# CODEJIN/multi_speaker_tts

Measured on AMD Instinct MI355X. Metric: mel-frames/sec (train step) at batch 32x(128 tok,800 mel), higher is better.
Workload: dtype f32

## Files before the change

multi_speaker_tts_amd/csrc/persist.hip:

```cpp
#include "persist_fwd_parts.h"

namespace mstts {

#ifndef M1_LATE
#define M1_LATE 60
#endif
#ifndef PRE_EARLY
#define PRE_EARLY 1
#endif
#ifndef SPLIT_M0
#define SPLIT_M0 1
#endif
#ifndef SPLIT_C0
#define SPLIT_C0 1
#endif

#ifndef FWD_QOWN
#define FWD_QOWN 1
#endif
#ifndef SPLIT_H1
#define SPLIT_H1 1
#endif
#ifndef SPLIT_H0
#define SPLIT_H0 1
#endif
#ifndef QP_LATE
#define QP_LATE 1
#endif
#ifndef QP_SLEEP
#define QP_SLEEP 12
#endif
#ifndef H0_LATE
#define H0_LATE 1
#endif
#ifndef H1_REQ_EARLY
#define H1_REQ_EARLY 1
#endif
#ifndef P0_EARLY
#define P0_EARLY 0
#endif

constexpr long XCTX = 8L * 128 * 24, XACT = 8L * 128 * 32, XPART = 256L * 8 * 2 * 256, XM1 = 32L * PH, XEN = 32L * 8 * PTMAX;
constexpr long OFF_CTX = 0, OFF_M0 = OFF_CTX + PRING * XCTX, OFF_H0 = OFF_M0 + PRING * XACT, OFF_H1 = OFF_H0 + PRING * XACT,
               OFF_M1 = OFF_H1 + PRING * XACT, OFF_EN = OFF_M1 + PRING * XM1, OFF_P0 = OFF_EN + PRING * XEN, OFF_P1 = OFF_P0 + PRING * XPART,
               OFF_QP = OFF_P1 + PRING * XPART, XQP = 32L * 8 * 256 * 16,
               XCH_FLOATS = OFF_QP + (FWD_QOWN ? PRING * XQP : 0);
template <int TT> struct FL {
    static constexpr int S_STG = 0, S_RED = S_STG + (TT == 128 ? 3 * 128 * 32 / 2 : 128 * LA),
                         S_TR = S_RED + 4 * 2 * 256, S_M1 = S_TR + 2 * 128,
                         S_EN = TT > 128 ? S_STG : S_M1 + PH, S_CUM = TT > 128 ? S_M1 + PH : S_EN + 8 * PT,
                         S_A = S_CUM + TT + 48, S_Q = S_A + TT, S_QF = S_Q + 512, S_CO = S_QF + 16, S_LK = S_CO + 4 * 96,
                         S_FLAG = S_LK + 32 * 16, S_STAMP = S_FLAG + 4, S_VAL = S_STAMP + 2 * 16, S_WQ = S_VAL + PT * 96, S_FLOATS = S_WQ + 8 * 512 * 4;
    static_assert(8 * TT <= 128 * LA && S_FLOATS * 4 <= 160 * 1024, "LDS budget");
};
constexpr int NSTAMP = 16;

struct PersistFwd {
    const float* w0pk; const float* w1pk; const float* wqpk;
    const float* xw0; const float* b1;
    const float* pre; const float* b0;
    const uint8_t* zc0; const uint8_t* zh0; const uint8_t* zc1; const uint8_t* zh1; float keep;
    const float* keys; const float* values; const int32_t* lengths;
    const float* loc_k; const float* loc_b; const float* score_w; const float* score_b;
    int B, S, T;
    float* in0; float* in1; float* pj; float* c0; float* c1; float* acts0; float* acts1; float* craw0; float* craw1;
    float* q_hist; float* align_hist; float* cum_hist;
    float* opk;
    float* xch; unsigned* ctrl;
    unsigned long long* stamps;
    int fail_step; int near_xcd;
};


template <bool PROF, bool FOLD, int TT, bool BF16 = false>
__global__ __launch_bounds__(PTH) void persist_fwd_kernel(PersistFwd d) {
    static_assert(!BF16 || FOLD, "the bf16 instantiation forms the prenet rows' product itself");
    constexpr bool SM0 = SPLIT_M0 && !BF16 && FOLD && TT == 128;
    constexpr bool PE = PRE_EARLY && SPLIT_M0 && SPLIT_C0 && !BF16 && FOLD && TT == 128;
    constexpr bool SC0 = SPLIT_C0 && SM0;
    constexpr bool QO = FWD_QOWN && SC0, SH1 = SPLIT_H1 && QO, SH0 = SPLIT_H0 && QO;
    constexpr int S_BIA = FL<TT>::S_Q + 128;
    typedef FL<TT> Y;
    constexpr int S_STG = Y::S_STG, S_RED = Y::S_RED, S_TR = Y::S_TR, S_M1 = Y::S_M1, S_EN = Y::S_EN, S_CUM = Y::S_CUM, S_A = Y::S_A, S_Q = Y::S_Q,
                  S_CO = Y::S_CO, S_LK = Y::S_LK, S_FLAG = Y::S_FLAG, S_STAMP = Y::S_STAMP, S_VAL = Y::S_VAL, S_WQ = Y::S_WQ;
    constexpr int S_WQO = S_M1, S_W1LO = S_WQ, S_W0LO = S_WQ + 4 * 512 * 4;
    constexpr int NH = TT / 128;
    extern __shared__ __attribute__((aligned(16))) float sm[];
    const int g0 = blockIdx.x, tid0 = threadIdx.x, wave0 = __builtin_amdgcn_readfirstlane(tid0 >> 6);
    int g = g0, gi = g & 7, gj = g >> 3;
    int tid = tid0, lane = tid & 63, wave = wave0;
    const int B = d.B, S = d.S, T = d.T;
    const __amdgpu_buffer_rsrc_t xr = __builtin_amdgcn_make_buffer_rsrc(d.xch, 0, (int)(XCH_FLOATS * 4), 0x00020000);
    unsigned* sflag = reinterpret_cast<unsigned*>(sm + S_FLAG);
    float* stg = sm + S_STG;
    __bf16* stg16 = reinterpret_cast<__bf16*>(sm + S_STG);

    if (d.near_xcd) persist_scrub(xr, OFF_CTX, OFF_M1 - OFF_CTX, g0, tid);
    __syncthreads();
    if (tid == 0) {
// ... 23 lines not shown
    }
    pbf16x8 w1s[SM0 ? 3 : 1][SM0 ? 4 : 1];
    pbf16x8 w0s[SC0 ? 3 : 1][SC0 ? 4 : 1];
    if constexpr (SM0) {
        const float* p1 = d.w1pk + ((long)(g * 8 + wave) * 64) * 64 + lane;
        const float* p0 = d.w0pk + ((long)(g * 8 + wave) * 64) * 64 + lane;
#pragma unroll
        for (int r = 0; r < 32; ++r) {
            {
                const float x = p1[r * 64];
                const __bf16 hi = (__bf16)x; const float r1 = x - (float)hi;
                const __bf16 mid = (__bf16)r1; const float r2 = r1 - (float)mid;
                w1s[0][r >> 3][r & 7] = hi; w1s[1][r >> 3][r & 7] = mid; w1s[2][r >> 3][r & 7] = (__bf16)r2;
            }
            if constexpr (SC0) {
                const float x = p0[r * 64];
                const __bf16 hi = (__bf16)x; const float r1 = x - (float)hi;
                const __bf16 mid = (__bf16)r1; const float r2 = r1 - (float)mid;
                w0s[0][r >> 3][r & 7] = hi; w0s[1][r >> 3][r & 7] = mid; w0s[2][r >> 3][r & 7] = (__bf16)r2;
            }
        }
    }
    pbf16x8 w1h[SH1 ? 2 : 1][SH1 ? 4 : 1];
    pbf16x8 w0h[SH0 ? 2 : 1][SH0 ? 4 : 1];
    if constexpr (SH1 || SH0) {
        const float* p1 = d.w1pk + ((long)(g * 8 + wave) * 64) * 64 + lane;
        const float* p0 = d.w0pk + ((long)(g * 8 + wave) * 64) * 64 + lane;
#pragma unroll
        for (int j = 0; j < 4; ++j) {
            pbf16x8 lo1, lo0;
#pragma unroll
// ... 15 lines not shown
            if constexpr (SH0) *reinterpret_cast<pbf16x8*>(sm + S_W0LO + (j * PTH + tid) * 4) = lo0;
        }
    }
    int ab = gj;
    const bool arow = ab < B;
    const int alen = arow ? (d.lengths ? d.lengths[ab] : T) : 0;
    int ak = tid & 15, atg = tid >> 4;
    float kreg[4 * NH];
    float asb = 0.f, awk = 0.f;
    {
#pragma unroll
        for (int m = 0; m < 4 * NH; ++m) {
            const int t = 128 * (m >> 2) + 4 * atg + (m & 3);
            kreg[m] = (arow && t < T) ? d.keys[((long)ab * T + t) * PA + 16 * gi + ak] : 0.f;
        }
        asb = d.score_b[16 * gi + ak] + d.loc_b[16 * gi + ak];
        awk = d.score_w[16 * gi + ak];
        if constexpr (SC0) {
            if (tid < 16) { sm[S_BIA + 32 + tid] = asb; sm[S_BIA + 48 + tid] = awk; }
            if (tid < 32) {
                const int q = (tid >> 2) & 3, u = 4 * g + (tid & 3);
                sm[S_BIA + tid] = (tid < 16) ? d.b0[q * PH + u] : d.b1[q * PH + u];
            }
        }
        for (int x = tid; x < 32 * 16; x += PTH) sm[S_LK + x] = (x < PKS * 16) ? d.loc_k[(x >> 4) * PA + 16 * gi + (x & 15)] : 0.f;
        for (int x = tid; x < PT * 96; x += PTH) {
            const int t = x / 96, c = x - t * 96;
            sm[S_VAL + x] = (arow && t < alen && t < T) ? d.values[((long)ab * T + t) * PM + 96 * gi + c] : 0.f;
        }
        for (int x = tid; x < TT + 48; x += PTH) sm[S_CUM + x] = 0.f;
        if constexpr (QO) {
            if (tid < 128) {
                const pf32x4 v = reinterpret_cast<const pf32x4*>(d.wqpk)[((long)(tid >> 4) * 8 + gi) * 512 + 16 * gj + (tid & 15)];
#pragma unroll
                for (int u = 0; u < 4; ++u) sm[S_WQO + u * 128 + tid] = v[u];
            }
        } else {
            const pf32x4* wqs = reinterpret_cast<const pf32x4*>(d.wqpk) + (long)gi * 8 * 512;
            for (int x = tid; x < 8 * 512; x += PTH) {
                pf32x4 v = wqs[x];
                if constexpr (BF16) { v[0] = bf16_round(v[0]); v[1] = bf16_round(v[1]); v[2] = bf16_round(v[2]); v[3] = bf16_round(v[3]); }
                reinterpret_cast<pf32x4*>(sm + S_WQ)[x] = v;
            }
// ... 29 lines not shown
    if (wave < 4) {                                                                                                             \
        _Pragma("unroll") for (int m = 0; m < 4; ++m)                                                                           \
            poff[m] = (unsigned)(((OFFP) + slot * XPART + (((long)g * 8 + 2 * wave + (m >> 1)) * 2 + (m & 1)) * 256) * 4 + 16 * lane); \
        issue<4>(xr, poff, pv);                                                                                                 \
    }
#define COMPLETE_PARTIALS()                                                                                                     \
    if (wave < 4) {                                                                                                             \
        const unsigned gens__[4] = {gen, gen, gen, gen};                                                                        \
        if (!complete<4>(xr, poff, pv, d.ctrl, gens__)) PFAIL();                                                                        \
        *reinterpret_cast<pf32x4*>(sm + S_RED + ((wave * 2 + 0) * 64 + lane) * 4) = pv[0] + pv[2];                              \
        *reinterpret_cast<pf32x4*>(sm + S_RED + ((wave * 2 + 1) * 64 + lane) * 4) = pv[1] + pv[3];                              \
    }
#define SUM_PARTIALS()                                                                                                          \
    ((*reinterpret_cast<const pf32x4*>(sm + S_RED + ((0 * 2 + et) * 64 + lane) * 4) + *reinterpret_cast<const pf32x4*>(sm + S_RED + ((1 * 2 + et) * 64 + lane) * 4)) + \
     (*reinterpret_cast<const pf32x4*>(sm + S_RED + ((2 * 2 + et) * 64 + lane) * 4) + *reinterpret_cast<const pf32x4*>(sm + S_RED + ((3 * 2 + et) * 64 + lane) * 4)))
    __syncthreads();
    if (PROF && tid == 0) sflag[2] = (unsigned)wall_clock64();

    float xwv[4] = {0.f, 0.f, 0.f, 0.f};
    pf32x4 prv = {0.f, 0.f, 0.f, 0.f};
    uint8_t zc0v, zh0v, zc1v, zh1v;
#define PL_TID (QO ? tid : tid0)
#define PL_WAVE (QO ? wave : wave0)
#define PL_G (QO ? g : g0)
#define LOAD_PRE(ST) do { const long bp__ = (long)(ST) * B;                                                                                  \
            const unsigned rho__ = ((unsigned)PL_TID & 255u) >> 1, pb__ = 16 * ((rho__ >> 4) & 1u) + (rho__ & 15u);                                     \
            const pf32x4 v__ = *reinterpret_cast<const pf32x4*>(d.pre + (bp__ + (pb__ < (unsigned)B ? pb__ : 0u)) * 256 + 32 * (PL_G & 7) + 8 * (rho__ >> 5) + 4 * ((unsigned)PL_TID & 1u)); \
            prv = pb__ < (unsigned)B ? v__ : (pf32x4){0.f, 0.f, 0.f, 0.f}; } while (0)
#define LOAD_OPERANDS(ST) do { const long b__ = (long)(ST) * B; const unsigned r__ = (16 * (PL_WAVE & 1) + (PL_TID & 15)) < (unsigned)B ? 16 * (PL_WAVE & 1) + (PL_TID & 15) : 0u;  \
         \
// ... 33 lines not shown
                __syncthreads();
                mfma_part_bf16<3, 4, 0>(wb0, stg16, lane, acc0);
            } else if constexpr (SC0) {
                if (!PE || s == 0) {
                    if (tid < 256) sp3_put_rk(stg16, tid >> 1, 6 + (tid & 1), prv);
                    __syncthreads();
                    mfma_part_split3<3, 4>(w0s, stg16, lane, acc0);
                }
            } else {
                if (tid < 256) *reinterpret_cast<pf32x4*>(stg + (tid >> 1) * LA + 24 + 4 * (tid & 1)) = prv;
                __syncthreads();
                mfma_part<6, 8, LA, 0, 64>(w0, stg, lane, acc0);
            }
            if (s > 0) {
                PSTAMP(0);
                slice_issue<6>(xr, OFF_CTX + pslot * XCTX + gi * 3072L, tid, soff, sv);
                if constexpr (BF16) { if (!slice_complete_bf16<6>(xr, stg16, tid, soff, sv, d.ctrl, pgen)) PFAIL(); }
                else if constexpr (SC0) { if (!slice_complete_split3_k6(xr, stg16, tid, soff, sv, d.ctrl, pgen)) PFAIL(); }
                else { if (!slice_complete<6, LA>(xr, stg, tid, soff, sv, d.ctrl, pgen)) PFAIL(); }
                PABORT_CHECK();
                PSTAMP(1);
                if constexpr (BF16) mfma_part_bf16<0, 3, 0>(wb0, stg16, lane, acc0);
                else if constexpr (SC0) mfma_part_split3<0, 3>(w0s, stg16, lane, acc0);
                else mfma_part<0, 6, LA, 0, 64>(w0, stg, lane, acc0);
            }
        } else {
            if (s > 0) {
                PSTAMP(0);
                slice_issue<6>(xr, OFF_CTX + pslot * XCTX + gi * 3072L, tid, soff, sv);
                if (!slice_complete<6, LC>(xr, stg, tid, soff, sv, d.ctrl, pgen)) PFAIL();
                PABORT_CHECK();
                PSTAMP(1);
            }
            if constexpr (!BF16) { if (s > 0) mfma_part<0, 6, LC, 0, 64>(w0, stg, lane, acc0); }
        }
        if constexpr (SH1 && H1_REQ_EARLY) { if (s > 0) slice_issue<8>(xr, OFF_H1 + pslot * XACT + gi * 4096L, tid, soff, sv); }
        PUBLISH_PARTIAL(OFF_P0, acc0)
        PSTAMP(2);
        if (s > 0) {
            if constexpr (!(SH1 && H1_REQ_EARLY)) slice_issue<8>(xr, OFF_H1 + pslot * XACT + gi * 4096L, tid, soff, sv);
            __syncthreads();
            if constexpr (BF16) { if (!slice_complete_bf16<8>(xr, stg16, tid, soff, sv, d.ctrl, pgen)) PFAIL(); }
            else if constexpr (SH1) { if (!slice_complete_split3(xr, stg16, tid, soff, sv, d.ctrl, pgen)) PFAIL(); }
            else { if (!slice_complete<8, LA>(xr, stg, tid, soff, sv, d.ctrl, pgen)) PFAIL(); }
            PABORT_CHECK();
            if constexpr (SH1 && P0_EARLY) { ISSUE_PARTIALS(OFF_P0) }
            if constexpr (BF16) mfma_part_bf16<0, 4, 4>(wb1, stg16, lane, acc1);
            else if constexpr (SH1) mfma_part_split3_lds<0, 4>(w1h, sm + S_W1LO + 4 * tid, stg16, lane, acc1);
            else mfma_part<0, 8, LA, 32, 64>(w1, stg, lane, acc1);
        }
        PSTAMP(13);
        if (!(SH1 && P0_EARLY) || s == 0) { ISSUE_PARTIALS(OFF_P0) }
        COMPLETE_PARTIALS()
        PABORT_CHECK();
        PSTAMP(3);
        {
            const pf32x4 gs = SUM_PARTIALS();
            float add0[4];
#pragma unroll
            for (int q = 0; q < 4; ++q) add0[q] = SC0 ? sm[S_BIA + q * 4 + ee] : FOLD ? b0v[q] : (rowok ? xwv[q] : 0.f);
            const float cprev0 = c0s;
            const CellOut o = cell_update(gs, add0, c0s, h0s, (zc0v || !rowok) ? d.keep : 0.f, (zh0v || !rowok) ? d.keep : 0.f);
            if (ew) {
                sm[S_TR + er * 4 + ee] = o.m;
                sm[S_TR + 128 + er * 4 + ee] = h0s;
            }
            __syncthreads();
            if (tid < 64) {
                const int arr = tid >> 5, row = tid & 31;
                const pf32x4 val = *reinterpret_cast<const pf32x4*>(sm + S_TR + arr * 128 + row * 4);
                const int rho = (((gj & 3) * 2 + (row >> 4)) * 16) + (row & 15);
                const long base = arr ? OFF_H0 : OFF_M0;
                const long o2 = gi * 4096L + rho * 32 + 4 * (gj >> 2);
                xpublish_near(xr, (unsigned)((base + slot * XACT + o2) * 4), val, gen, near);
            }
// ... 161 lines not shown
                if (lane < 16) sm[S_Q + wave * 16 + lane] = qp;
            }
            }
            __syncthreads();
            float qsum = 0.f;
#pragma unroll
            for (int u = 0; u < 8; ++u) qsum += sm[S_Q + u * 16 + ak];
            if (tid < 16) (d.q_hist + (sB + ab) * PA + 16 * gi)[tid] = qsum;
            {
                const float qk = qsum + (SC0 ? sm[S_BIA + 32 + ak] : asb);
#pragma unroll
                for (int hh = 0; hh < NH; ++hh) {
                    const pf32x4 loc = locv[hh];
                    float pre[4];
#pragma unroll
                    for (int m = 0; m < 4; ++m) pre[m] = kreg[4 * hh + m] + qk + loc[m];
                    pf32x4 e4;
#pragma unroll
                    for (int m = 0; m < 4; ++m) {
                        float e = (SC0 ? sm[S_BIA + 48 + ak] : awk) * tanhf_(pre[m]);
                        e += dpp_mov<0xB1, 0xf>(0.f, e);
                        e += dpp_mov<0x4E, 0xf>(0.f, e);
                        e += dpp_mov<0x141, 0xf>(0.f, e);
                        e += dpp_mov<0x140, 0xf>(0.f, e);
                        e4[m] = e;
                    }
                    if (ak == 0) {
                        const long o = ((long)ab * 8 + gi) * TT + 128 * hh + 4 * atg;
                        xpublish(xr, (unsigned)((OFF_EN + slot * XEN + o) * 4), e4, gen);
                    }
                }
// ... 31 lines not shown
                mx = wave_max(mx);
                float ps = 0.f;
#pragma unroll
                for (int i = 0; i < 2 * NH; ++i) { ev[i] = (lane + 64 * i < alen) ? __expf(ev[i] - mx) : 0.f; ps += ev[i]; }
                const float inv = 1.f / wave_sum(ps);
                float* ah = d.align_hist + (sB + ab) * T; float* ch = d.cum_hist + (sB1 + ab) * T;
#pragma unroll
                for (int i = 0; i < 2 * NH; ++i) {
                    const float a = ev[i] * inv, n = sm[S_CUM + 15 + 64 * i + lane] + a;
                    sm[S_A + 64 * i + lane] = a;
                    sm[S_CUM + 15 + 64 * i + lane] = n;
                    if (gi == 0 && lane + 64 * i < T) { ah[lane + 64 * i] = a; ch[lane + 64 * i] = n; }
                }
            }
            __syncthreads();
            if (tid < 384) {
                const int c = tid % 96, th = tid / 96;
                float acc = 0.f;
#pragma unroll
                for (int t4 = 0; t4 < 8; ++t4) {
                    const pf32x4 a4 = *reinterpret_cast<const pf32x4*>(sm + S_A + 32 * th + 4 * t4);
#pragma unroll
                    for (int e = 0; e < 4; ++e) acc += a4[e] * sm[S_VAL + (32 * th + 4 * t4 + e) * 96 + c];
                }
                if (NH > 1) {
                    const float* vg = d.values + ((long)ab * T + 128 + 32 * th) * PM + 96 * gi + c;
                    const int nt = T - (128 + 32 * th) < 32 ? (T - (128 + 32 * th) > 0 ? T - (128 + 32 * th) : 0) : 32;
#pragma unroll 16
                    for (int t = 0; t < 32; ++t) acc += sm[S_A + 128 + 32 * th + t] * (t < nt ? vg[(long)t * PM] : 0.f);
                }
                sm[S_CO + th * 96 + c] = acc;
            }
            __syncthreads();
            if (tid < 24) {
                const pf32x4 val = (*reinterpret_cast<const pf32x4*>(sm + S_CO + 4 * tid) + *reinterpret_cast<const pf32x4*>(sm + S_CO + 96 + 4 * tid)) +
                                   (*reinterpret_cast<const pf32x4*>(sm + S_CO + 192 + 4 * tid) + *reinterpret_cast<const pf32x4*>(sm + S_CO + 288 + 4 * tid));
                const int qq = tid / 6, k4 = tid - qq * 6;
                const int rho = ((qq * 2 + (ab >> 4)) * 16) + (ab & 15);
                const long o = gi * 3072L + rho * 24 + 4 * k4;
                xpublish_near(xr, (unsigned)((OFF_CTX + slot * XCTX + o) * 4), val, gen, near);
                reinterpret_cast<pf32x4*>(d.in0 + (sB1 + ab) * (PM + PH) + 96 * gi)[tid] = val;
                reinterpret_cast<pf32x4*>(d.pj + (sB + ab) * (PH + PM) + PH + 96 * gi)[tid] = val;
            }
        } else {
            PSTAMP(14);
            if (tid < 24) {
                const int qq = tid / 6, k4 = tid - qq * 6;
                const int rho = ((qq * 2 + (ab >> 4)) * 16) + (ab & 15);
                const long o = gi * 3072L + rho * 24 + 4 * k4;
                xpublish_near(xr, (unsigned)((OFF_CTX + slot * XCTX + o) * 4), (pf32x4){0.f, 0.f, 0.f, 0.f}, gen, near);
            }
        }
        PSTAMP(15);
        LOAD_OPERANDS(s + 1 < S ? s + 1 : s);
    }
    if (tid == 0) {
        __hip_atomic_fetch_add(d.ctrl + 2, 1u, __ATOMIC_RELAXED, __HIP_MEMORY_SCOPE_AGENT);
        if (PROF && d.stamps) {
#pragma unroll
            for (int x = 0; x < NSTAMP; ++x) d.stamps[(long)g * NSTAMP + x] = sstamp[x];
        }
    }
#undef PSTAMP
#undef LOAD_OPERANDS
#undef LOAD_PRE
#undef PL_TID
#undef PL_WAVE
#undef PL_G
#undef PABORT_CHECK
#undef PFAIL
#undef PUBLISH_PARTIAL
#undef ISSUE_PARTIALS
#undef COMPLETE_PARTIALS
#undef SUM_PARTIALS
}


__global__ void persist_pack_cells_kernel(const float* __restrict__ w0f, const float* __restrict__ w1, const float* __restrict__ wx0, float* __restrict__ w0pk, float* __restrict__ w1pk) {
    const long n0 = 256L * 8 * 64 * 64, n1 = 256L * 8 * 64 * 64;
    for (long p = blockIdx.x * (long)blockDim.x + threadIdx.x; p < n0 + n1; p += (long)gridDim.x * blockDim.x) {
        const bool c1 = p >= n0;
        long r = c1 ? p - n0 : p;
        const int lane = (int)(r & 63); r >>= 6;
        const int ks = (int)(r & 63); r >>= 6;
        const int wave = (int)(r & 7), g = (int)(r >> 3);
        const int gi = g & 7, gj = g >> 3;
        const int q = lane >> 4, mcol = lane & 15, ue = mcol >> 2, gate = mcol & 3;
        const int u = 32 * gj + 4 * wave + ue;
        const long col = (long)gate * PH + u;
        long row;
        if (!c1) row = ks < 24 ? 96 * gi + 24 * q + ks : ks < 32 ? 32 * gi + 8 * q + (ks - 24) : PM + unit_of_kstep(gi, ks - 32, q);
        else row = ks < 32 ? unit_of_kstep(gi, ks, q) : PH + unit_of_kstep(gi, ks - 32, q);
        if (c1) w1pk[p - n0] = w1[row * 4 * PH + col];
        else w0pk[p] = (ks >= 24 && ks < 32) ? (wx0 ? wx0[row * 4 * PH + col] : 0.f) : w0f[row * 4 * PH + col];
    }
}
__global__ void persist_pack_wq_kernel(const float* __restrict__ wq, float* __restrict__ wqpk) {
    const int p = blockIdx.x * blockDim.x + threadIdx.x;
    if (p >= 8 * 64 * 256) return;
    const int e = p & 3, tid = (p >> 2) & 511, x4 = (p >> 11) & 7, gi = p >> 14;
    wqpk[p] = wq[(long)(32 * (tid >> 4) + 4 * x4 + e) * PA + 16 * gi + (tid & 15)];
}

}
using namespace mstts;

#define PFW_INST(P_, F_, T_, B16_) {persist_fwd_kernel<P_, F_, T_, B16_>, (int)(FL<T_>::S_FLOATS * 4)}
#define PFW_FORMS(T_)                                                                                                                  \
    PFW_INST(false, false, T_, false), PFW_INST(true, false, T_, false), PFW_INST(false, true, T_, false), PFW_INST(true, true, T_, false), \
    PFW_INST(false, true, T_, true), PFW_INST(true, true, T_, true)
static const PersistInst<PersistFwd> FWD_TABLE[] = {PFW_FORMS(128), PFW_FORMS(256)};
#undef PFW_FORMS
#undef PFW_INST
constexpr int fwd_index(bool t256, int form, bool stamps) { return (t256 * 3 + form) * 2 + stamps; }
static_assert(sizeof(FWD_TABLE) / sizeof(FWD_TABLE[0]) == fwd_index(true, 2, true) + 1, "one table row per (positions, form, stamps)");

extern "C" int64_t mstts_persist_fwd_ws_bytes(void) { return XCH_FLOATS * 4; }
extern "C" int64_t mstts_persist_pack_floats(int32_t which) { return which == 0 ? 256L * 8 * 64 * 64 : which == 1 ? 256L * 8 * 64 * 64 : 8L * 64 * 256; }

extern "C" int32_t mstts_persist_fwd_supported(int64_t B, int64_t H, int64_t M, int64_t A, int64_t T, int64_t KS) {
    if (!(B >= 1 && B <= PROWS && H == PH && M == PM && A == PA && T >= 1 && T <= PTMAX && KS == PKS)) return 0;
    static int memo[PERSIST_MAX_DEVICES];
    return persist_device_memo(memo, [](int dev) { return persist_probe(dev, FWD_TABLE); });
}

extern "C" int mstts_persist_pack(const float* w0f, const float* w1, const float* wq, const float* wx0, float* w0pk, float* w1pk, float* wqpk, mstts_stream_t s) {
    MSTTS_REQUIRE(w0f && w1 && wq && w0pk && w1pk && wqpk, MSTTS_ERR_SHAPE, "persist_pack: null pointer");
    hipLaunchKernelGGL(persist_pack_cells_kernel, dim3(4096), dim3(256), 0, (hipStream_t)s, w0f, w1, wx0, w0pk, w1pk);
    MSTTS_CHECK_LAUNCH("persist_pack_cells");
    hipLaunchKernelGGL(persist_pack_wq_kernel, dim3(8 * 64), dim3(256), 0, (hipStream_t)s, wq, wqpk);
    MSTTS_CHECK_LAUNCH("persist_pack_wq");
    return MSTTS_OK;
}

extern "C" int mstts_decoder_train_fwd_persistent(const mstts_decoder_train_desc* d, const mstts_persist_desc* p, mstts_stream_t s) {
    const bool fold = p && p->pre != nullptr;
    MSTTS_REQUIRE(d && p && (fold ? p->b0 != nullptr : d->xw0 != nullptr) && d->b1 && d->in0 && d->in1 && d->pj && d->c0 && d->c1 && d->acts0 && d->acts1 && d->craw0 && d->craw1 &&
                  d->q_hist && d->align_hist && d->cum_hist && p->w0pk && p->w1pk && p->wqpk && p->xch && p->ctrl, MSTTS_ERR_SHAPE,
                  "decoder_train_fwd_persistent: null pointer");
    const long B = d->B, S = d->S, H = d->H, M = d->lsa.M, A = d->lsa.A, T = d->lsa.T;
    MSTTS_REQUIRE(d->lsa.B == B && mstts_persist_fwd_supported(B, H, M, A, T, d->lsa.KS), MSTTS_ERR_SHAPE,
                  "decoder_train_fwd_persistent: shape or device not supported (see mstts_persist_fwd_supported)");
    MSTTS_REQUIRE(d->zc0 && d->zh0 && d->zc1 && d->zh1, MSTTS_ERR_SHAPE, "decoder_train_fwd_persistent: the four zoneout keep-masks are required (all ones = no zoneout)");
    MSTTS_REQUIRE(d->lsa.keys && d->lsa.values && d->lsa.loc_k && d->lsa.loc_b && d->lsa.score_w && d->lsa.score_b, MSTTS_ERR_SHAPE,
                  "decoder_train_fwd_persistent: attention constants missing");
    MSTTS_REQUIRE(aligned16(p->xch) && aligned16(d->in0) && aligned16(d->pj) && (M + H) % 4 == 0, MSTTS_ERR_ALIGN, "decoder_train_fwd_persistent: 16-byte alignment");
    hipStream_t hs = (hipStream_t)s;
    hipError_t e = hipMemsetAsync(d->in0, 0, B * (M + H) * sizeof(float), hs);
    if (e == hipSuccess) e = hipMemsetAsync(d->in1, 0, B * 2 * H * sizeof(float), hs);
    if (e == hipSuccess) e = hipMemsetAsync(d->c0, 0, B * H * sizeof(float), hs);
    if (e == hipSuccess) e = hipMemsetAsync(d->c1, 0, B * H * sizeof(float), hs);
    if (e == hipSuccess) e = hipMemsetAsync(d->cum_hist, 0, B * T * sizeof(float), hs);
    if (e != hipSuccess) return set_err(MSTTS_ERR_LAUNCH, "decoder_train_fwd_persistent: memset: %s", hipGetErrorString(e));
    if (int r = persist_arm("decoder_train_fwd_persistent", p->xch, XCH_FLOATS * 4, p->ctrl, PCTRL_WORDS, hs)) return r;
    PersistFwd a;
    MSTTS_REQUIRE(!fold || (d->P == 256 && aligned16(p->pre)), MSTTS_ERR_SHAPE, "decoder_train_fwd_persistent: the folded prenet product needs a 256-wide prenet, 16-byte aligned");
    a.w0pk = p->w0pk; a.w1pk = p->w1pk; a.wqpk = p->wqpk; a.xw0 = d->xw0; a.b1 = d->b1; a.pre = p->pre; a.b0 = p->b0;
    a.zc0 = d->zc0; a.zh0 = d->zh0; a.zc1 = d->zc1; a.zh1 = d->zh1; a.keep = 1.f - d->zoneout;
    a.keys = d->lsa.keys; a.values = d->lsa.values; a.lengths = d->lsa.lengths;
    a.loc_k = d->lsa.loc_k; a.loc_b = d->lsa.loc_b; a.score_w = d->lsa.score_w; a.score_b = d->lsa.score_b;
    a.B = (int)B; a.S = (int)S; a.T = (int)T;
    a.in0 = d->in0; a.in1 = d->in1; a.pj = d->pj; a.c0 = d->c0; a.c1 = d->c1; a.acts0 = d->acts0; a.acts1 = d->acts1;
    a.craw0 = d->craw0; a.craw1 = d->craw1; a.q_hist = d->q_hist; a.align_hist = d->align_hist; a.cum_hist = d->cum_hist;
    a.opk = p->opk; a.xch = p->xch; a.ctrl = p->ctrl; a.stamps = (unsigned long long*)p->stamps;
    persist_knobs(a, p->selftest_fail_step, p->near_xcd);
    MSTTS_REQUIRE(!p->recurrent_bf16 || fold, MSTTS_ERR_SHAPE, "decoder_train_fwd_persistent: the bf16 form needs the folded prenet product (pre / b0)");
    const PersistInst<PersistFwd>& k = FWD_TABLE[fwd_index(T > 128, p->recurrent_bf16 ? 2 : fold ? 1 : 0, p->stamps != nullptr)];
    hipLaunchKernelGGL(k.kernel, dim3(PWG), dim3(PTH), (size_t)k.lds_bytes, hs, a);
    MSTTS_CHECK_LAUNCH("persist_fwd");
    return MSTTS_OK;
}
```

multi_speaker_tts_amd/csrc/persist_fwd_parts.h:

```cpp
#pragma once
#include "persist_common.h"
#include "lstm_cell.h"

namespace mstts {

constexpr int LC = 28, LA = 36;

template <int K4A, int K4B, int LD, int WOFF, int NW, int NT = 2>
__device__ __forceinline__ void mfma_part(const float (&w)[NW], const float* sx, int lane, pf32x4 (&acc)[2]) {
    const int row0 = ((lane >> 4) * 2) * 16 + (lane & 15);
#pragma unroll
    for (int k4 = K4A; k4 < K4B; ++k4) {
        const pf32x4 x0 = *reinterpret_cast<const pf32x4*>(sx + row0 * LD + 4 * k4);
        if (NT == 2) {
            const pf32x4 x1 = *reinterpret_cast<const pf32x4*>(sx + (row0 + 16) * LD + 4 * k4);
#pragma unroll
            for (int e = 0; e < 4; ++e) {
                acc[0] = PMFMA(w[WOFF + 4 * k4 + e], x0[e], acc[0]);
                acc[1] = PMFMA(w[WOFF + 4 * k4 + e], x1[e], acc[1]);
            }
        } else {
#pragma unroll
            for (int e = 0; e < 4; ++e) acc[0] = PMFMA(w[WOFF + 4 * k4 + e], x0[e], acc[0]);
        }
// ... 82 lines not shown
}
__device__ __forceinline__ bool slice_complete_split3(__amdgpu_buffer_rsrc_t xr, __bf16* stg, int tid, const unsigned (&off)[2], pf32x4 (&v)[2], const unsigned* ctrl, unsigned gen) {
    const unsigned gens[2] = {gen, gen};
    const bool ok = complete<2>(xr, off, v, ctrl, gens);
    sp3_put(stg, tid, v[0]);
    sp3_put(stg, tid + PTH, v[1]);
    return ok;
}
__device__ __forceinline__ bool slice_complete_split3_k6(__amdgpu_buffer_rsrc_t xr, __bf16* stg, int tid, const unsigned (&off)[2], pf32x4 (&v)[2], const unsigned* ctrl, unsigned gen) {
    const unsigned gens[2] = {gen, gen};
    const bool ok = complete<2>(xr, off, v, ctrl, gens);
    { const int rho = tid / 6; sp3_put_rk(stg, rho, tid - rho * 6, v[0]); }
    if (tid + PTH < 128 * 6) { const int p = tid + PTH, rho = p / 6; sp3_put_rk(stg, rho, p - rho * 6, v[1]); }
    return ok;
}
template <int JA = 0, int JB = 4>
__device__ __forceinline__ void mfma_part_split3(const pbf16x8 (&wsp)[3][4], const __bf16* sx, int lane, pf32x4 (&acc)[2]) {
    const int row0 = ((lane >> 4) * 2) * 16 + (lane & 15);
#pragma unroll
    for (int j = JA; j < JB; ++j) {
#pragma unroll
        for (int t = 0; t < 2; ++t) {
            const __bf16* p = sx + sp3_off(row0 + 16 * t, j);
            const pbf16x8 xh = *reinterpret_cast<const pbf16x8*>(p), xm = *reinterpret_cast<const pbf16x8*>(p + SP3_PLANE),
                          xl = *reinterpret_cast<const pbf16x8*>(p + 2 * SP3_PLANE);
            acc[t] = PMFMA_BF16(wsp[0][j], xh, acc[t]);
            acc[t] = PMFMA_BF16(wsp[1][j], xh, acc[t]);
            acc[t] = PMFMA_BF16(wsp[0][j], xm, acc[t]);
            acc[t] = PMFMA_BF16(wsp[1][j], xm, acc[t]);
            acc[t] = PMFMA_BF16(wsp[2][j], xh, acc[t]);
// ... 40 lines not shown
```

multi_speaker_tts_amd/engine.py:

```python
from __future__ import annotations

import ctypes as C
import os
import types
import warnings

import numpy as np
import torch

from . import lib
from .lib import ACT_NONE, ACT_RELU, ACT_TANH, gemm, ptr, call
from .masks import MaskSet, step_seed
from .params import CELL, ENC_CELL, LSA, LSA_VARS, VOC, Dims, ParamStore, bank_groups, bank_suffix
from .persist import PERSIST_COOLDOWN, PERSIST_STRIKES, CoolDown, Ticket, decoder_workgroups, lstm_bwd_workgroups, lstm_fwd_workgroups, near_xcd
from .training import (BN_EPS, BN_MOM, Engine, _split_k, _split_k_big, bn_train_fwd, conv_bn_bwd, conv_fwd, exponential_decay, lstm_layer_grads,
                       lstm_seq_bwd, lstm_seq_fwd)

MAX_PLANS = 64


def learning_rate(step):
    from . import Hyper_Parameters as hp
    return exponential_decay(hp.Train.Learning_Rate, step)

# ... 368 lines not shown
        w.d_pj = f(S, B, H + M, zero=bool(self.ctx_dead))
        w.dg0, w.dg1 = f(S, B, 4 * H), f(S, B, 4 * H)
        w.dq_hist, w.de_hist = f(S, B, A), f(S, B, Te)
        w.d_in0_parts = int(lb.mstts_decoder_train_bwd_parts(H, M))
        w.d_in0 = f(w.d_in0_parts, S, B, M + H, zero=bool(self.ctx_dead))
        w.dec_bwd_ws = f(int(lb.mstts_decoder_train_bwd_ws_floats(B, H, M, A, Te, d.att_ch)), zero=True)
        w.lsa_param_ws = f((int(lb.mstts_lsa_param_bwd_ws_floats(B, Te, S)) + 3) // 4 * 4)
        w.d_pre, w.d_pre2 = f(S * B, Pn), f(S * B, Pn)
        w.d_keys, w.d_values = f(B, Te, A), f(B, Te, M, zero=bool(self.ctx_dead))
        w.enc_dgs, w.enc_dgp = {dr: f(Te, B, 4 * He) for dr in ("fw", "bw")}, {dr: f(B, Te, 4 * He) for dr in ("fw", "bw")}
        w.enc_bwd_ws = {dr: f(int(lb.mstts_lstm_seq_ws_floats(B, He, 1))) for dr in ("fw", "bw")}
        w.enc_dy, w.enc_dz, w.enc_dx = f(B * Te, max(d.enc_conv_ch, d.emb)), f(B * Te, d.enc_conv_ch), f(B * Te, max(d.enc_conv_ch, d.emb))
        w.job_flag, w.job_flag_host = cv.take(1, dtype=torch.int32), self._pin("job_flag_host", 1)
        w.dec, w.dec_b = lib.DecoderTrain(), lib.DecoderTrainBwd()
        w.dec_b.ctx_dead = self.ctx_dead
        if w.persist_bwd:
            w.pdesc_b.ctx_dead = self.ctx_dead
        w.zero_on_activate, w.extent_bytes, w.arena_generation = cv.zero, cv.off, self._arena.generation
        return (None if (cv.count or cv.overflow) else w), cv.off

    def _forward_plan(self, w, batch, masks, allowed, overlap_vocoder, redo):
        allowed = False if redo else (self._persist_begin_step() if allowed is None else bool(allowed))
        decoder, bptt, encoder = bool(w.persist) and allowed, bool(w.persist_bwd) and allowed, bool(w.persist_enc) and allowed
        return types.SimpleNamespace(
            decoder=decoder,
            bptt=bptt,
            packed_bptt=decoder and bptt,
            encoder=encoder,
            encoder_forked=encoder and ENC_OVERLAP,
            late_masks=masks is None and encoder and ENC_OVERLAP,
# ... 612 lines not shown
```

Baseline: 669,500.

## Specialize persistent decoder forward for constant dead context columns

When the last 256 value channels are constant over time (ctx_dead), a new kernel instantiation computes the attention context only over the live channels. A small pre-kernel folds the dead channels' contribution into a per-batch cell-0 gate constant, and another kernel fills the dead columns of in0/pj. This shrinks the per-step context exchange and MFMA work, and the change also enables early partial issue with an 8-wave reduction layout. In exchange it adds two launches, extra LDS use for keys and the constant, and a more complex weight-loading path.

```diff
diff --git a/multi_speaker_tts_amd/csrc/persist.hip b/multi_speaker_tts_amd/csrc/persist.hip
--- a/multi_speaker_tts_amd/csrc/persist.hip
+++ b/multi_speaker_tts_amd/csrc/persist.hip
@@ -37,8 +37,9 @@
 #define H1_REQ_EARLY 1
 #endif
 #ifndef P0_EARLY
-#define P0_EARLY 0
-#endif
+#define P0_EARLY 2
+#endif
+constexpr bool FWD_LIVE_BUILT = FWD_QOWN && SPLIT_C0 && SPLIT_M0;
 
 constexpr long XCTX = 8L * 128 * 24, XACT = 8L * 128 * 32, XPART = 256L * 8 * 2 * 256, XM1 = 32L * PH, XEN = 32L * 8 * PTMAX;
 constexpr long OFF_CTX = 0, OFF_M0 = OFF_CTX + PRING * XCTX, OFF_H0 = OFF_M0 + PRING * XACT, OFF_H1 = OFF_H0 + PRING * XACT,
@@ -61,6 +62,7 @@
     const float* pre; const float* b0;
     const uint8_t* zc0; const uint8_t* zh0; const uint8_t* zc1; const uint8_t* zh1; float keep;
     const float* keys; const float* values; const int32_t* lengths;
+    const float* cst;
     const float* loc_k; const float* loc_b; const float* score_w; const float* score_b;
     int B, S, T;
     float* in0; float* in1; float* pj; float* c0; float* c1; float* acts0; float* acts1; float* craw0; float* craw1;
@@ -72,17 +74,23 @@
 };
 
 
-template <bool PROF, bool FOLD, int TT, bool BF16 = false>
+template <bool PROF, bool FOLD, int TT, bool BF16 = false, int MC = PM>
 __global__ __launch_bounds__(PTH) void persist_fwd_kernel(PersistFwd d) {
     static_assert(!BF16 || FOLD, "the bf16 instantiation forms the prenet rows' product itself");
+    constexpr bool LIVE = MC != PM;
+    constexpr int CW = MC / 8, K4C = CW / 16;
+    static_assert(MC == PM || (MC == PM - 256 && FWD_LIVE_BUILT && !BF16 && FOLD && TT == 128), "live width: the fp32 / folded / 128-position instantiation only");
     constexpr bool SM0 = SPLIT_M0 && !BF16 && FOLD && TT == 128;
     constexpr bool PE = PRE_EARLY && SPLIT_M0 && SPLIT_C0 && !BF16 && FOLD && TT == 128;
     constexpr bool SC0 = SPLIT_C0 && SM0;
     constexpr bool QO = FWD_QOWN && SC0, SH1 = SPLIT_H1 && QO, SH0 = SPLIT_H0 && QO;
+    constexpr bool P0E = P0_EARLY && SH1 && LIVE, P0E8 = P0E && P0_EARLY == 2;
     constexpr int S_BIA = FL<TT>::S_Q + 128;
     typedef FL<TT> Y;
     constexpr int S_STG = Y::S_STG, S_RED = Y::S_RED, S_TR = Y::S_TR, S_M1 = Y::S_M1, S_EN = Y::S_EN, S_CUM = Y::S_CUM, S_A = Y::S_A, S_Q = Y::S_Q,
                   S_CO = Y::S_CO, S_LK = Y::S_LK, S_FLAG = Y::S_FLAG, S_STAMP = Y::S_STAMP, S_VAL = Y::S_VAL, S_WQ = Y::S_WQ;
+    constexpr int S_KEY = S_VAL + PT * CW;
+    constexpr int S_CST = S_M1 + 512;
     constexpr int S_WQO = S_M1, S_W1LO = S_WQ, S_W0LO = S_WQ + 4 * 512 * 4;
     constexpr int NH = TT / 128;
     extern __shared__ __attribute__((aligned(16))) float sm[];
@@ -136,7 +144,9 @@
                 w1s[0][r >> 3][r & 7] = hi; w1s[1][r >> 3][r & 7] = mid; w1s[2][r >> 3][r & 7] = (__bf16)r2;
             }
             if constexpr (SC0) {
-                const float x = p0[r * 64];
+                const int crow = 64 * gi + 16 * (lane >> 4) + r, ci = crow / 96, cq = (crow - 96 * ci) / 24, ck = crow - 96 * ci - 24 * cq;
+                const float x = (!LIVE || r >= 24) ? p0[r * 64] : r >= 16 ? 0.f
+                              : d.w0pk[((long)((gj * 8 + ci) * 8 + wave) * 64 + ck) * 64 + 16 * cq + (lane & 15)];
                 const __bf16 hi = (__bf16)x; const float r1 = x - (float)hi;
                 const __bf16 mid = (__bf16)r1; const float r2 = r1 - (float)mid;
                 w0s[0][r >> 3][r & 7] = hi; w0s[1][r >> 3][r & 7] = mid; w0s[2][r >> 3][r & 7] = (__bf16)r2;
@@ -182,6 +192,7 @@
             const int t = 128 * (m >> 2) + 4 * atg + (m & 3);
             kreg[m] = (arow && t < T) ? d.keys[((long)ab * T + t) * PA + 16 * gi + ak] : 0.f;
         }
+        if constexpr (LIVE) *reinterpret_cast<pf32x4*>(sm + S_KEY + 4 * tid) = (pf32x4){kreg[0], kreg[1], kreg[2], kreg[3]};
         asb = d.score_b[16 * gi + ak] + d.loc_b[16 * gi + ak];
         awk = d.score_w[16 * gi + ak];
         if constexpr (SC0) {
@@ -192,9 +203,13 @@
             }
         }
         for (int x = tid; x < 32 * 16; x += PTH) sm[S_LK + x] = (x < PKS * 16) ? d.loc_k[(x >> 4) * PA + 16 * gi + (x & 15)] : 0.f;
-        for (int x = tid; x < PT * 96; x += PTH) {
-            const int t = x / 96, c = x - t * 96;
-            sm[S_VAL + x] = (arow && t < alen && t < T) ? d.values[((long)ab * T + t) * PM + 96 * gi + c] : 0.f;
+        for (int x = tid; x < PT * CW; x += PTH) {
+            const int t = x / CW, c = x - t * CW;
+            sm[S_VAL + x] = (arow && t < alen && t < T) ? d.values[((long)ab * T + t) * PM + CW * gi + c] : 0.f;
+        }
+        if constexpr (LIVE) {
+            const int r = tid & 31;
+            sm[S_CST + tid] = r < B ? d.cst[(long)r * 4 * PH + (tid >> 7) * PH + 4 * g + ((tid >> 5) & 3)] : 0.f;
         }
         for (int x = tid; x < TT + 48; x += PTH) sm[S_CUM + x] = 0.f;
         if constexpr (QO) {
@@ -254,6 +269,19 @@
 #define SUM_PARTIALS()                                                                                                          \
     ((*reinterpret_cast<const pf32x4*>(sm + S_RED + ((0 * 2 + et) * 64 + lane) * 4) + *reinterpret_cast<const pf32x4*>(sm + S_RED + ((1 * 2 + et) * 64 + lane) * 4)) + \
      (*reinterpret_cast<const pf32x4*>(sm + S_RED + ((2 * 2 + et) * 64 + lane) * 4) + *reinterpret_cast<const pf32x4*>(sm + S_RED + ((3 * 2 + et) * 64 + lane) * 4)))
+#define S_RED8(W) ((W) < 4 ? S_RED + (W) * 512 : S_KEY + 2048 + ((W) - 4) * 512)
+#define ISSUE_PARTIALS8(OFFP) do {                                                                                              \
+        _Pragma("unroll") for (int m = 0; m < 2; ++m)                                                                           \
+            soff[m] = (unsigned)(((OFFP) + slot * XPART + (((long)g * 8 + wave) * 2 + m) * 256) * 4 + 16 * lane);               \
+        issue<2>(xr, soff, sv); } while (0)
+#define COMPLETE_PARTIALS8() do {                                                                                               \
+        const unsigned gens__[2] = {gen, gen};                                                                                  \
+        if (!complete<2>(xr, soff, sv, d.ctrl, gens__)) PFAIL();                                                                \
+        float* red__ = sm + (wave < 4 ? S_RED + wave * 512 : S_KEY + 2048 + (wave - 4) * 512);                                  \
+        *reinterpret_cast<pf32x4*>(red__ + lane * 4) = sv[0];                                                                   \
+        *reinterpret_cast<pf32x4*>(red__ + (64 + lane) * 4) = sv[1]; } while (0)
+#define RED8(W) (*reinterpret_cast<const pf32x4*>(sm + S_RED8(W) + (et * 64 + lane) * 4))
+#define SUM_PARTIALS8() (((RED8(0) + RED8(1)) + (RED8(2) + RED8(3))) + ((RED8(4) + RED8(5)) + (RED8(6) + RED8(7))))
     __syncthreads();
     if (PROF && tid == 0) sflag[2] = (unsigned)wall_clock64();
 
@@ -317,13 +345,16 @@
             }
             if (s > 0) {
                 PSTAMP(0);
-                slice_issue<6>(xr, OFF_CTX + pslot * XCTX + gi * 3072L, tid, soff, sv);
+                if constexpr (LIVE) slice_issue_k4(xr, OFF_CTX + pslot * XCTX + gi * (128L * CW / 4), tid, soff, sv);
+                else slice_issue<6>(xr, OFF_CTX + pslot * XCTX + gi * 3072L, tid, soff, sv);
                 if constexpr (BF16) { if (!slice_complete_bf16<6>(xr, stg16, tid, soff, sv, d.ctrl, pgen)) PFAIL(); }
+                else if constexpr (LIVE) { if (!slice_complete_split3_k4(xr, stg16, tid, soff, sv, d.ctrl, pgen)) PFAIL(); }
                 else if constexpr (SC0) { if (!slice_complete_split3_k6(xr, stg16, tid, soff, sv, d.ctrl, pgen)) PFAIL(); }
                 else { if (!slice_complete<6, LA>(xr, stg, tid, soff, sv, d.ctrl, pgen)) PFAIL(); }
                 PABORT_CHECK();
                 PSTAMP(1);
                 if constexpr (BF16) mfma_part_bf16<0, 3, 0>(wb0, stg16, lane, acc0);
+                else if constexpr (LIVE) mfma_part_split3<0, 2>(w0s, stg16, lane, acc0);
                 else if constexpr (SC0) mfma_part_split3<0, 3>(w0s, stg16, lane, acc0);
                 else mfma_part<0, 6, LA, 0, 64>(w0, stg, lane, acc0);
             }
@@ -347,21 +378,33 @@
             else if constexpr (SH1) { if (!slice_complete_split3(xr, stg16, tid, soff, sv, d.ctrl, pgen)) PFAIL(); }
             else { if (!slice_complete<8, LA>(xr, stg, tid, soff, sv, d.ctrl, pgen)) PFAIL(); }
             PABORT_CHECK();
-            if constexpr (SH1 && P0_EARLY) { ISSUE_PARTIALS(OFF_P0) }
+            if constexpr (P0E8) ISSUE_PARTIALS8(OFF_P0);
+            else if constexpr (P0E) { ISSUE_PARTIALS(OFF_P0) }
             if constexpr (BF16) mfma_part_bf16<0, 4, 4>(wb1, stg16, lane, acc1);
             else if constexpr (SH1) mfma_part_split3_lds<0, 4>(w1h, sm + S_W1LO + 4 * tid, stg16, lane, acc1);
             else mfma_part<0, 8, LA, 32, 64>(w1, stg, lane, acc1);
         }
         PSTAMP(13);
-        if (!(SH1 && P0_EARLY) || s == 0) { ISSUE_PARTIALS(OFF_P0) }
-        COMPLETE_PARTIALS()
+        if constexpr (P0E8) {
+            if (s == 0) ISSUE_PARTIALS8(OFF_P0);
+            COMPLETE_PARTIALS8();
+        } else {
+            if (!P0E || s == 0) { ISSUE_PARTIALS(OFF_P0) }
+            COMPLETE_PARTIALS()
+        }
         PABORT_CHECK();
         PSTAMP(3);
         {
-            const pf32x4 gs = SUM_PARTIALS();
+            const pf32x4 gs = P0E8 ? SUM_PARTIALS8() : SUM_PARTIALS();
             float add0[4];
 #pragma unroll
             for (int q = 0; q < 4; ++q) add0[q] = SC0 ? sm[S_BIA + q * 4 + ee] : FOLD ? b0v[q] : (rowok ? xwv[q] : 0.f);
+            if constexpr (LIVE) {
+                if (s > 0) {
+#pragma unroll
+                    for (int q = 0; q < 4; ++q) add0[q] += sm[S_CST + (q * 4 + ee) * 32 + er];
+                }
+            }
             const float cprev0 = c0s;
             const CellOut o = cell_update(gs, add0, c0s, h0s, (zc0v || !rowok) ? d.keep : 0.f, (zh0v || !rowok) ? d.keep : 0.f);
             if (ew) {
@@ -553,7 +596,7 @@
                     const pf32x4 loc = locv[hh];
                     float pre[4];
 #pragma unroll
-                    for (int m = 0; m < 4; ++m) pre[m] = kreg[4 * hh + m] + qk + loc[m];
+                    for (int m = 0; m < 4; ++m) pre[m] = (LIVE ? sm[S_KEY + 4 * tid + m] : kreg[4 * hh + m]) + qk + loc[m];
                     pf32x4 e4;
 #pragma unroll
                     for (int m = 0; m < 4; ++m) {
@@ -615,40 +658,40 @@
                 }
             }
             __syncthreads();
-            if (tid < 384) {
-                const int c = tid % 96, th = tid / 96;
+            if (tid < 4 * CW) {
+                const int c = tid % CW, th = tid / CW;
                 float acc = 0.f;
 #pragma unroll
                 for (int t4 = 0; t4 < 8; ++t4) {
                     const pf32x4 a4 = *reinterpret_cast<const pf32x4*>(sm + S_A + 32 * th + 4 * t4);
 #pragma unroll
-                    for (int e = 0; e < 4; ++e) acc += a4[e] * sm[S_VAL + (32 * th + 4 * t4 + e) * 96 + c];
+                    for (int e = 0; e < 4; ++e) acc += a4[e] * sm[S_VAL + (32 * th + 4 * t4 + e) * CW + c];
                 }
                 if (NH > 1) {
-                    const float* vg = d.values + ((long)ab * T + 128 + 32 * th) * PM + 96 * gi + c;
+                    const float* vg = d.values + ((long)ab * T + 128 + 32 * th) * PM + CW * gi + c;
                     const int nt = T - (128 + 32 * th) < 32 ? (T - (128 + 32 * th) > 0 ? T - (128 + 32 * th) : 0) : 32;
 #pragma unroll 16
                     for (int t = 0; t < 32; ++t) acc += sm[S_A + 128 + 32 * th + t] * (t < nt ? vg[(long)t * PM] : 0.f);
                 }
-                sm[S_CO + th * 96 + c] = acc;
+                sm[S_CO + th * CW + c] = acc;
             }
             __syncthreads();
-            if (tid < 24) {
-                const pf32x4 val = (*reinterpret_cast<const pf32x4*>(sm + S_CO + 4 * tid) + *reinterpret_cast<const pf32x4*>(sm + S_CO + 96 + 4 * tid)) +
-                                   (*reinterpret_cast<const pf32x4*>(sm + S_CO + 192 + 4 * tid) + *reinterpret_cast<const pf32x4*>(sm + S_CO + 288 + 4 * tid));
-                const int qq = tid / 6, k4 = tid - qq * 6;
+            if (tid < CW / 4) {
+                const pf32x4 val = (*reinterpret_cast<const pf32x4*>(sm + S_CO + 4 * tid) + *reinterpret_cast<const pf32x4*>(sm + S_CO + CW + 4 * tid)) +
+                                   (*reinterpret_cast<const pf32x4*>(sm + S_CO + 2 * CW + 4 * tid) + *reinterpret_cast<const pf32x4*>(sm + S_CO + 3 * CW + 4 * tid));
+                const int qq = tid / K4C, k4 = tid - qq * K4C;
                 const int rho = ((qq * 2 + (ab >> 4)) * 16) + (ab & 15);
-                const long o = gi * 3072L + rho * 24 + 4 * k4;
+                const long o = gi * (128L * CW / 4) + rho * (CW / 4) + 4 * k4;
                 xpublish_near(xr, (unsigned)((OFF_CTX + slot * XCTX + o) * 4), val, gen, near);
-                reinterpret_cast<pf32x4*>(d.in0 + (sB1 + ab) * (PM + PH) + 96 * gi)[tid] = val;
-                reinterpret_cast<pf32x4*>(d.pj + (sB + ab) * (PH + PM) + PH + 96 * gi)[tid] = val;
+                reinterpret_cast<pf32x4*>(d.in0 + (sB1 + ab) * (PM + PH) + CW * gi)[tid] = val;
+                reinterpret_cast<pf32x4*>(d.pj + (sB + ab) * (PH + PM) + PH + CW * gi)[tid] = val;
             }
         } else {
             PSTAMP(14);
-            if (tid < 24) {
-                const int qq = tid / 6, k4 = tid - qq * 6;
+            if (tid < CW / 4) {
+                const int qq = tid / K4C, k4 = tid - qq * K4C;
                 const int rho = ((qq * 2 + (ab >> 4)) * 16) + (ab & 15);
-                const long o = gi * 3072L + rho * 24 + 4 * k4;
+                const long o = gi * (128L * CW / 4) + rho * (CW / 4) + 4 * k4;
                 xpublish_near(xr, (unsigned)((OFF_CTX + slot * XCTX + o) * 4), (pf32x4){0.f, 0.f, 0.f, 0.f}, gen, near);
             }
         }
@@ -674,6 +717,11 @@
 #undef ISSUE_PARTIALS
 #undef COMPLETE_PARTIALS
 #undef SUM_PARTIALS
+#undef S_RED8
+#undef ISSUE_PARTIALS8
+#undef COMPLETE_PARTIALS8
+#undef RED8
+#undef SUM_PARTIALS8
 }
 
 
@@ -703,20 +751,56 @@
     wqpk[p] = wq[(long)(32 * (tid >> 4) + 4 * x4 + e) * PA + 16 * gi + (tid & 15)];
 }
 
+constexpr int PDEAD = 256, PLIVE = PM - PDEAD;
+constexpr int CST_ROWS = 4;
+__global__ __launch_bounds__(256) void persist_ctx_const_kernel(const float* __restrict__ values, const float* __restrict__ w0f, float* __restrict__ cst, int B, int T) {
+    __shared__ float spk[CST_ROWS][PDEAD];
+    const int b0 = blockIdx.y * CST_ROWS, col = blockIdx.x * 256 + threadIdx.x;
+#pragma unroll
+    for (int r = 0; r < CST_ROWS; ++r) spk[r][threadIdx.x] = b0 + r < B ? values[(long)(b0 + r) * T * PM + PLIVE + threadIdx.x] : 0.f;
+    __syncthreads();
+    double acc[CST_ROWS] = {0., 0., 0., 0.};
+    const float* w = w0f + (long)PLIVE * 4 * PH + col;
+#pragma unroll 8
+    for (int k = 0; k < PDEAD; ++k) {
+        const double x = (double)w[(long)k * 4 * PH];
+#pragma unroll
+        for (int r = 0; r < CST_ROWS; ++r) acc[r] = fma((double)spk[r][k], x, acc[r]);
+    }
+#pragma unroll
+    for (int r = 0; r < CST_ROWS; ++r)
+        if (b0 + r < B) cst[(long)(b0 + r) * 4 * PH + col] = (float)acc[r];
+}
+__global__ void persist_fill_dead_kernel(const float* __restrict__ values, float* __restrict__ in0, float* __restrict__ pj, int B, int S, int T) {
+    const long n = (long)S * B * (PDEAD / 4);
+    for (long p = blockIdx.x * (long)blockDim.x + threadIdx.x; p < n; p += (long)gridDim.x * blockDim.x) {
+        const int c4 = (int)(p % (PDEAD / 4));
+        const long sb = p / (PDEAD / 4);
+        const int b = (int)(sb % B);
+        const pf32x4 v = *reinterpret_cast<const pf32x4*>(values + (long)b * T * PM + PLIVE + 4 * c4);
+        *reinterpret_cast<pf32x4*>(in0 + (sb + B) * (PM + PH) + PLIVE + 4 * c4) = v;
+        *reinterpret_cast<pf32x4*>(pj + sb * (PH + PM) + PH + PLIVE + 4 * c4) = v;
+    }
+}
+
 }
 using namespace mstts;
 
 #define PFW_INST(P_, F_, T_, B16_) {persist_fwd_kernel<P_, F_, T_, B16_>, (int)(FL<T_>::S_FLOATS * 4)}
+#define PFW_LIVE(P_) {persist_fwd_kernel<P_, true, 128, false, FWD_LIVE_BUILT ? PLIVE : PM>, (int)(FL<128>::S_FLOATS * 4)}
 #define PFW_FORMS(T_)                                                                                                                  \
     PFW_INST(false, false, T_, false), PFW_INST(true, false, T_, false), PFW_INST(false, true, T_, false), PFW_INST(true, true, T_, false), \
     PFW_INST(false, true, T_, true), PFW_INST(true, true, T_, true)
-static const PersistInst<PersistFwd> FWD_TABLE[] = {PFW_FORMS(128), PFW_FORMS(256)};
+static const PersistInst<PersistFwd> FWD_TABLE[] = {PFW_FORMS(128), PFW_FORMS(256), PFW_LIVE(false), PFW_LIVE(true)};
 #undef PFW_FORMS
+#undef PFW_LIVE
 #undef PFW_INST
 constexpr int fwd_index(bool t256, int form, bool stamps) { return (t256 * 3 + form) * 2 + stamps; }
-static_assert(sizeof(FWD_TABLE) / sizeof(FWD_TABLE[0]) == fwd_index(true, 2, true) + 1, "one table row per (positions, form, stamps)");
-
-extern "C" int64_t mstts_persist_fwd_ws_bytes(void) { return XCH_FLOATS * 4; }
+constexpr int FWD_LIVE = fwd_index(true, 2, true) + 1;
+static_assert(sizeof(FWD_TABLE) / sizeof(FWD_TABLE[0]) == FWD_LIVE + 2, "one table row per (positions, form, stamps), then the live-width pair");
+
+constexpr long XCST_FLOATS = (long)PROWS * 4 * PH;
+extern "C" int64_t mstts_persist_fwd_ws_bytes(void) { return (XCH_FLOATS + XCST_FLOATS) * 4; }
 extern "C" int64_t mstts_persist_pack_floats(int32_t which) { return which == 0 ? 256L * 8 * 64 * 64 : which == 1 ? 256L * 8 * 64 * 64 : 8L * 64 * 256; }
 
 extern "C" int32_t mstts_persist_fwd_supported(int64_t B, int64_t H, int64_t M, int64_t A, int64_t T, int64_t KS) {
@@ -746,6 +830,9 @@
     MSTTS_REQUIRE(d->lsa.keys && d->lsa.values && d->lsa.loc_k && d->lsa.loc_b && d->lsa.score_w && d->lsa.score_b, MSTTS_ERR_SHAPE,
                   "decoder_train_fwd_persistent: attention constants missing");
     MSTTS_REQUIRE(aligned16(p->xch) && aligned16(d->in0) && aligned16(d->pj) && (M + H) % 4 == 0, MSTTS_ERR_ALIGN, "decoder_train_fwd_persistent: 16-byte alignment");
+    MSTTS_REQUIRE(p->ctx_dead == 0 || p->ctx_dead == PDEAD, MSTTS_ERR_SHAPE, "decoder_train_fwd_persistent: ctx_dead must be 0 or 256");
+    const bool live = p->ctx_dead == PDEAD && FWD_LIVE_BUILT && fold && !p->recurrent_bf16 && T <= 128;
+    MSTTS_REQUIRE(!live || (d->w0f && aligned16(d->lsa.values)), MSTTS_ERR_SHAPE, "decoder_train_fwd_persistent: ctx_dead needs the folded cell-0 kernel w0f and 16-byte aligned values");
     hipStream_t hs = (hipStream_t)s;
     hipError_t e = hipMemsetAsync(d->in0, 0, B * (M + H) * sizeof(float), hs);
     if (e == hipSuccess) e = hipMemsetAsync(d->in1, 0, B * 2 * H * sizeof(float), hs);
@@ -766,7 +853,14 @@
     a.opk = p->opk; a.xch = p->xch; a.ctrl = p->ctrl; a.stamps = (unsigned long long*)p->stamps;
     persist_knobs(a, p->selftest_fail_step, p->near_xcd);
     MSTTS_REQUIRE(!p->recurrent_bf16 || fold, MSTTS_ERR_SHAPE, "decoder_train_fwd_persistent: the bf16 form needs the folded prenet product (pre / b0)");
-    const PersistInst<PersistFwd>& k = FWD_TABLE[fwd_index(T > 128, p->recurrent_bf16 ? 2 : fold ? 1 : 0, p->stamps != nullptr)];
+    a.cst = p->xch + XCH_FLOATS;
+    if (live && S * B > 0) {
+        hipLaunchKernelGGL(persist_ctx_const_kernel, dim3(4 * PH / 256, (unsigned)((B + CST_ROWS - 1) / CST_ROWS)), dim3(256), 0, hs, a.values, d->w0f, p->xch + XCH_FLOATS, (int)B, (int)T);
+        MSTTS_CHECK_LAUNCH("persist_ctx_const");
+        hipLaunchKernelGGL(persist_fill_dead_kernel, dim3((unsigned)std::min<long>((S * B * (PDEAD / 4) + 255) / 256, 4096)), dim3(256), 0, hs, a.values, d->in0, d->pj, (int)B, (int)S, (int)T);
+        MSTTS_CHECK_LAUNCH("persist_fill_dead");
+    }
+    const PersistInst<PersistFwd>& k = FWD_TABLE[live ? FWD_LIVE + (p->stamps != nullptr) : fwd_index(T > 128, p->recurrent_bf16 ? 2 : fold ? 1 : 0, p->stamps != nullptr)];
     hipLaunchKernelGGL(k.kernel, dim3(PWG), dim3(PTH), (size_t)k.lds_bytes, hs, a);
     MSTTS_CHECK_LAUNCH("persist_fwd");
     return MSTTS_OK;
diff --git a/multi_speaker_tts_amd/csrc/persist_fwd_parts.h b/multi_speaker_tts_amd/csrc/persist_fwd_parts.h
--- a/multi_speaker_tts_amd/csrc/persist_fwd_parts.h
+++ b/multi_speaker_tts_amd/csrc/persist_fwd_parts.h
@@ -120,6 +120,19 @@
     if (tid + PTH < 128 * 6) { const int p = tid + PTH, rho = p / 6; sp3_put_rk(stg, rho, p - rho * 6, v[1]); }
     return ok;
 }
+__device__ __forceinline__ void slice_issue_k4(__amdgpu_buffer_rsrc_t xr, long slice_float_off, int tid, unsigned (&off)[2], pf32x4 (&v)[2]) {
+    unsigned o1[1] = {(unsigned)(slice_float_off * 4 + 16 * tid)};
+    pf32x4 v1[1];
+    issue<1>(xr, o1, v1);
+    off[0] = o1[0]; v[0] = v1[0];
+}
+__device__ __forceinline__ bool slice_complete_split3_k4(__amdgpu_buffer_rsrc_t xr, __bf16* stg, int tid, const unsigned (&off)[2], pf32x4 (&v)[2], const unsigned* ctrl, unsigned gen) {
+    const unsigned gens[1] = {gen}, o1[1] = {off[0]};
+    pf32x4 v1[1] = {v[0]};
+    const bool ok = complete<1>(xr, o1, v1, ctrl, gens);
+    sp3_put_rk(stg, tid >> 2, tid & 3, v1[0]);
+    return ok;
+}
 template <int JA = 0, int JB = 4>
 __device__ __forceinline__ void mfma_part_split3(const pbf16x8 (&wsp)[3][4], const __bf16* sx, int lane, pf32x4 (&acc)[2]) {
     const int row0 = ((lane >> 4) * 2) * 16 + (lane & 15);
diff --git a/multi_speaker_tts_amd/engine.py b/multi_speaker_tts_amd/engine.py
--- a/multi_speaker_tts_amd/engine.py
+++ b/multi_speaker_tts_amd/engine.py
@@ -406,6 +406,8 @@
         w.job_flag, w.job_flag_host = cv.take(1, dtype=torch.int32), self._pin("job_flag_host", 1)
         w.dec, w.dec_b = lib.DecoderTrain(), lib.DecoderTrainBwd()
         w.dec_b.ctx_dead = self.ctx_dead
+        if w.persist:
+            w.pdesc.ctx_dead = self.ctx_dead
         if w.persist_bwd:
             w.pdesc_b.ctx_dead = self.ctx_dead
         w.zero_on_activate, w.extent_bytes, w.arena_generation = cv.zero, cv.off, self._arena.generation
```

After: 677,400, median of 6. +1.2%, better.
